# ltiao/bore

Measured on AMD Instinct MI355X. Metric: BO-iterations/sec (fit+argmax), 16-16-1 MLP, higher is better.
Workload: dtype f32; 1 GPU; BASELINE config 4 (= config 1 x independent loops): Branin-2D, 16-16-1 MLP, q=0.25, 200 epochs, batch 64, 3 L-BFGS-B restarts from 1024 samples; loops_per_gpu=512, total_loops=512, schedule=async, N_start=15, N_end=217, parallelism=replica-shard x1

## Files before the change

### bore_amd/csrc/bore_engine.hip

```cpp
#include <hip/hip_runtime.h>

#include <chrono>
#include <cmath>
#include <cstdint>
#include <cstdlib>
#include <cstring>
#include <atomic>
#include <initializer_list>
#include <mutex>
#include <new>
#include <thread>
#include <vector>

#include <sched.h>

#include "../../include/bore_hip.h"
#include "host_common.h"

namespace {

struct Mt19937 {
  uint32_t key[624];
  int pos;
  uint32_t next32() {
    if (pos >= 624) {
      int i;
      for (i = 0; i < 624 - 397; ++i) {
        const uint32_t y = (key[i] & 0x80000000u) | (key[i + 1] & 0x7fffffffu);
        key[i] = key[i + 397] ^ (y >> 1) ^ (-(int32_t)(y & 1) & 0x9908b0dfu);
      }
      for (; i < 623; ++i) {
        const uint32_t y = (key[i] & 0x80000000u) | (key[i + 1] & 0x7fffffffu);
        key[i] = key[i + (397 - 624)] ^ (y >> 1) ^ (-(int32_t)(y & 1) & 0x9908b0dfu);
      }
      const uint32_t y = (key[623] & 0x80000000u) | (key[0] & 0x7fffffffu);
      key[623] = key[396] ^ (y >> 1) ^ (-(int32_t)(y & 1) & 0x9908b0dfu);
      pos = 0;
    }
    uint32_t y = key[pos++];
    y ^= (y >> 11);
    y ^= (y << 7) & 0x9d2c5680u;
    y ^= (y << 15) & 0xefc60000u;
    y ^= (y >> 18);
    return y;
  }
  double next_double() {
    const uint32_t a = next32() >> 5, b = next32() >> 6;
    return (a * 67108864.0 + b) / 9007199254740992.0;
  }
};

struct Group {
  int a = 0, b = 0;
  hipStream_t stream = nullptr;
  hipEvent_t done = nullptr, ev[4] = {nullptr, nullptr, nullptr, nullptr};
  int64_t n = 0, cap = 0;
  int64_t epochs_seen = 0, draws = 0, steps = 0;
  bool inflight = false, has_new = false;
  double *X_seen = nullptr, *y_seen = nullptr, *y_dense = nullptr;
  float *X32 = nullptr, *z = nullptr;
  double *new_x = nullptr, *new_y = nullptr;
  double *x0 = nullptr, *x = nullptr, *jac = nullptr, *fun = nullptr, *x_best = nullptr;
  int32_t *idx = nullptr, *info = nullptr, *best = nullptr;
  double *new_x_pin = nullptr, *new_y_pin = nullptr, *x_best_pin = nullptr;
  int32_t *best_pin = nullptr, *info_pin = nullptr;
};

struct Async {
  int64_t cap = 0;
  IterEngine eng = {};
  double *result = nullptr;
  int32_t *flag = nullptr;
  int64_t *stamps = nullptr;
  double ns_per_tick = 10.0;
  std::vector<int32_t> it, target, state;
  std::vector<double> x_new, y_new, ready_since;
  std::vector<double> seen_at;
  double *ynew = nullptr;
  int32_t *yseq = nullptr, *parked = nullptr;
  int32_t *abort_flag = nullptr;
  int64_t wait_ticks = 0;
  std::vector<uint8_t> via_launch;
  std::vector<Worker> workers;
  std::vector<int> scratch_ids, done_ids;
  std::vector<double> cb_x, cb_y;
  bool fused = false;
  bool queue = false;
  QueueEntry *q_ring = nullptr;
  unsigned long long *q_head = nullptr, q_tail = 0;
  unsigned long long *q_tail_host = nullptr;
  int q_mask = 0, q_wgs = 0;
  int per_cu = 0;
  int host_threads = 1;
  int32_t *d_ident = nullptr;
  std::vector<int> q_owner;
  long long n_resident = 0, n_parked = 0;
  int stream_concurrency = 0;
  std::vector<double> launched_at;
  std::vector<double> loop_acc;
  double sum_wait = 0, sum_flight = 0;
  long long n_wait = 0, n_batches = 0, n_slots = 0;
};

}

__global__ void bore_spin_kernel(long long ticks) {
  const long long t0 = wall_clock64();
  while (wall_clock64() - t0 < ticks) __builtin_amdgcn_s_sleep(8);
}

extern "C" int bore_objective_branin01(const double *x, int64_t n, int32_t D, double *y, void *) {
  if (D != 2 || !x || !y) return 1;
  const double pi = 3.141592653589793;
  const double a = 5.1 / (4 * (pi * pi)), b = 5 / pi, c = 10 * (1 - 1 / (8 * pi));
  for (int64_t i = 0; i < n; ++i) {
    const double x1 = 15.0 * x[2 * i] - 5.0, x2 = 15.0 * x[2 * i + 1];
    const double t = x2 - a * (x1 * x1) + b * x1 - 6;
    y[i] = t * t + c * std::cos(x1) + 10;
  }
  return 0;
}

struct bore_engine {
  bore_mlp_desc desc;
  bore_engine_cfg cfg;
  int D = 0, P = 0;
  std::vector<double> low, high;
  bore_objective_fn objective = nullptr;
  void *user = nullptr;
  float *theta = nullptr, *adam_m = nullptr, *adam_v = nullptr;
  int64_t *adam_t = nullptr;
  std::vector<Mt19937> rs;
  std::vector<Group> groups;
  bore_engine_stats st;
  std::vector<double> y_tmp;
  Async *as = nullptr;
  bool poisoned = false;
};

namespace {

double now_s() {
  return std::chrono::duration<double>(std::chrono::steady_clock::now().time_since_epoch()).count();
}

template <typename T>
int dev_alloc(T **p, size_t count) {
  HIP_TRY(hipMalloc(reinterpret_cast<void **>(p), count * sizeof(T)));
  return 0;
}
template <typename T>
int pin_alloc(T **p, size_t count) {
  HIP_TRY(hipHostMalloc(reinterpret_cast<void **>(p), count * sizeof(T), hipHostMallocDefault));
  return 0;
// ... 218 lines not shown
  return 0;
}

int async_create(bore_engine *e, const double *X0, const double *y0) {
  const size_t L = e->cfg.n_loops, D = e->D, R = e->cfg.num_starts, n0 = e->cfg.n_init;
  if (R > 16) return fail(BORE_E_UNSUPPORTED, "engine_create: async_loops needs num_starts <= 16");
  e->as = new (std::nothrow) Async();
  if (!e->as) return fail(BORE_E_HIP, "engine_create: out of memory");
  Async &A = *e->as;
  int rc;
  if ((rc = async_alloc(e, n0 * 2 > 128 ? n0 * 2 : 128))) return rc;
  {
    const bore_engine_cfg &c = e->cfg;
    IterEngine &E = A.eng;
    E.desc = &e->desc; E.theta = e->theta; E.adam_m = e->adam_m; E.adam_v = e->adam_v; E.adam_t = e->adam_t;
    E.gamma = c.gamma; E.epochs = c.epochs; E.batch_size = c.batch_size; E.seed = c.seed; E.loop_id0 = c.loop_id0;
    E.adam = &c.adam; E.num_samples = c.num_samples; E.low = e->low.data(); E.high = e->high.data();
    E.num_starts = c.num_starts; E.transform = c.transform; E.opts = &c.lbfgsb; E.n_loops = c.n_loops;
  }
  std::vector<float> x32(L * n0 * D);
  for (size_t i = 0; i < x32.size(); ++i) x32[i] = (float)X0[i];
  HIP_TRY(hipMemcpy2D(A.eng.X_seen, A.cap * D * 8, X0, n0 * D * 8, n0 * D * 8, L, hipMemcpyHostToDevice));
  HIP_TRY(hipMemcpy2D(A.eng.y_seen, A.cap * 8, y0, n0 * 8, n0 * 8, L, hipMemcpyHostToDevice));
  HIP_TRY(hipMemcpy2D(A.eng.X32, A.cap * D * 4, x32.data(), n0 * D * 4, n0 * D * 4, L, hipMemcpyHostToDevice));
  if ((rc = pin_alloc(&A.result, L * (D + 8))) || (rc = pin_alloc(&A.flag, L)) ||
      (rc = dev_alloc(&A.stamps, L * 4)))
    return rc;
  std::memset(A.flag, 0, L * 4);
  HIP_TRY(hipMemset(A.stamps, 0, L * 4 * 8));
  {
    int dev = 0, khz = 0;
    HIP_TRY(hipGetDevice(&dev));
    if (hipDeviceGetAttribute(&khz, hipDeviceAttributeWallClockRate, dev) == hipSuccess && khz > 0)
      A.ns_per_tick = 1e6 / khz;
  }
  A.seen_at.assign(L, 0.0);
  A.via_launch.assign(L, 1);
  {
    char *blk = nullptr;
    const size_t bytes = L * (D + 1) * 8 + (2 * L + 1) * 4;
    if ((rc = pin_alloc(&blk, bytes))) return rc;
    std::memset(blk, 0, bytes);
    A.ynew = reinterpret_cast<double *>(blk);
    A.yseq = reinterpret_cast<int32_t *>(blk + L * (D + 1) * 8);
    A.parked = A.yseq + L;
    A.abort_flag = A.parked + L;
    for (size_t l = 0; l < L; ++l) A.parked[l] = -1;
  }
  A.it.assign(L, 0); A.target.assign(L, 0); A.state.assign(L, 2);
  A.x_new.assign(L * D, 0.0); A.y_new.assign(L, 0.0); A.ready_since.assign(L, 0.0);
  A.scratch_ids.reserve(L); A.cb_x.resize(L * D); A.cb_y.resize(L);
  A.launched_at.assign(L, 0.0);
  A.done_ids.assign(L, 0);
  A.fused = iteration_shape(&e->desc) != 0;
  const double resident_us = e->cfg.resident_wait_us < 0 ? 2000.0 : (double)e->cfg.resident_wait_us;
  A.wait_ticks = A.fused && resident_us > 0 ? (int64_t)(resident_us * 1e3 / A.ns_per_tick) : 0;
  const int queues = getenv("GPU_MAX_HW_QUEUES") ? atoi(getenv("GPU_MAX_HW_QUEUES")) : 4;
  int n_workers = A.fused ? 12 : 4;
  if (A.fused && n_workers > queues - 2) n_workers = queues - 2 > 2 ? queues - 2 : 2;
  if (e->cfg.worker_streams > 0) n_workers = e->cfg.worker_streams;
  A.workers.resize(n_workers > 0 ? n_workers : 1);
  for (Worker &w : A.workers) {
    HIP_TRY(hipStreamCreateWithFlags(&w.stream, hipStreamNonBlocking));
    HIP_TRY(hipEventCreateWithFlags(&w.done, hipEventDisableTiming));
    for (hipEvent_t &ev : w.ev) HIP_TRY(hipEventCreate(&ev));
    w.stage_bytes = ((sizeof(IterArgs) + 15) & ~(size_t)15) + L * (D + 1) * 8 + 3 * L * 4;
    char *hb = nullptr, *db = nullptr;
    if ((rc = pin_alloc(&hb, w.stage_bytes)) || (rc = dev_alloc(&db, w.stage_bytes))) return rc;
    const size_t o_dbl = (sizeof(IterArgs) + 15) & ~(size_t)15, o_int = o_dbl + L * (D + 1) * 8;
    w.h_args = reinterpret_cast<IterArgs *>(hb); w.d_args = reinterpret_cast<IterArgs *>(db);
    w.h_dbl = reinterpret_cast<double *>(hb + o_dbl); w.d_dbl = reinterpret_cast<double *>(db + o_dbl);
    w.h_int = reinterpret_cast<int32_t *>(hb + o_int); w.d_int = reinterpret_cast<int32_t *>(db + o_int);
    if ((rc = dev_alloc(&w.x0, L * R * D)) || (rc = dev_alloc(&w.x, L * R * D)) ||
        (rc = dev_alloc(&w.jac, L * R * D)) || (rc = dev_alloc(&w.fun, L * R)) ||
        (rc = dev_alloc(&w.idx, L * R)) || (rc = dev_alloc(&w.info, L * R * 5)))
      return rc;
  }
  if (A.workers.size() > 1) {
    const long long ticks = (long long)(2e6 / A.ns_per_tick);
    hipLaunchKernelGGL(bore_spin_kernel, dim3(1), dim3(64), 0, A.workers[0].stream, 1000LL);
    HIP_TRY(hipStreamSynchronize(A.workers[0].stream));
    double t0 = now_s();
    hipLaunchKernelGGL(bore_spin_kernel, dim3(1), dim3(64), 0, A.workers[0].stream, ticks);
    HIP_TRY(hipStreamSynchronize(A.workers[0].stream));
    const double one = now_s() - t0;
    t0 = now_s();
    for (Worker &w : A.workers) hipLaunchKernelGGL(bore_spin_kernel, dim3(1), dim3(64), 0, w.stream, ticks);
    for (Worker &w : A.workers) HIP_TRY(hipStreamSynchronize(w.stream));
    const double dt = now_s() - t0;
    int conc = (int)A.workers.size();
    if (dt > 1.5 * one) conc = (int)(A.workers.size() * one / dt + 0.5);
    conc = conc < 1 ? 1 : (conc > (int)A.workers.size() ? (int)A.workers.size() : conc);
    A.stream_concurrency = conc;
    if (conc < (int)A.workers.size()) {
      if (queues < (int)A.workers.size() + 2)
        fprintf(stderr,
                "bore_engine: %zu worker streams, but the device ran only about %d of them at once (one 2-ms probe "
                "alone %.2f ms, %zu at once %.2f ms): streams share hardware queues.  Set GPU_MAX_HW_QUEUES >= %zu in "
                "the environment BEFORE the first GPU call of the process (it is %d now).\n",
                A.workers.size(), conc, 1e3 * one, A.workers.size(), 1e3 * dt, A.workers.size() + 2, queues);
      else if (getenv("BORE_ASYNC_DEBUG"))
        fprintf(stderr,
                "bore_engine: stream probe: one 2-ms probe alone %.2f ms, %zu at once %.2f ms -> about %d run side by "
                "side (GPU_MAX_HW_QUEUES = %d already covers the %zu streams: not a queue shortage)\n",
                1e3 * one, A.workers.size(), 1e3 * dt, conc, queues, A.workers.size());
    }
  }
  return async_decide_schedule(e);
}

void async_destroy(bore_engine *e) {
  if (!e->as) return;
  Async &A = *e->as;
  for (Worker &w : A.workers) {
    free_all({w.d_args, w.x0, w.x, w.jac, w.fun, w.idx, w.info}, {w.h_args});
    free_stream(w.stream, w.done, w.ev);
  }
  free_all({A.eng.X_seen, A.eng.y_seen, A.eng.X32, A.eng.z, A.stamps, A.q_head, A.d_ident},
           {A.result, A.flag, A.ynew, A.q_ring, A.q_tail_host});
  delete e->as;
  e->as = nullptr;
}

int async_enqueue(bore_engine *e, Worker &w, int B, int64_t N_max) {
  const IterEngine &E = e->as->eng;
  void *sp = w.stream;
  int rc;
  if (e->as->fused) {
    if ((rc = record_event(w.ev[2], w.stream)) || (rc = iteration_launch(E, w, B)) || (rc = record_event(w.ev[3], w.stream)))
      return rc;
    return record_event(w.done, w.stream);
  }
  if ((rc = bore_append_observations(B, e->D, E.X_seen, E.y_seen, 0, e->as->cap, w.d_dbl,
                                     w.d_dbl + (size_t)E.n_loops * e->D, E.X32, nullptr, sp)) ||
      (rc = bore_labels(B, E.y_seen, N_max, E.gamma, E.z, nullptr, sp)) || (rc = record_event(w.ev[0], w.stream)) ||
      (rc = bore_mlp_fit(E.desc, B, E.theta, E.adam_m, E.adam_v, E.adam_t, E.X32, E.z, N_max, E.epochs, E.batch_size,
                         nullptr, E.seed, E.loop_id0, 0, E.adam, nullptr, sp)) ||
      (rc = record_event(w.ev[1], w.stream)) ||
      (rc = bore_sample_screen_topk(E.desc, B, E.theta, E.seed, E.loop_id0, 0, E.num_samples, E.low, E.high,
                                    E.num_starts, w.x0, w.idx, nullptr, sp)) ||
      (rc = record_event(w.ev[2], w.stream)) ||
      (rc = bore_lbfgsb_minimize(E.desc, B, E.theta, E.transform, 1, w.x0, E.num_starts, E.low, E.high, E.opts, w.x,
                                 w.fun, w.jac, w.info, sp)) ||
      (rc = record_event(w.ev[3], w.stream)))
    return rc;
  return record_event(w.done, w.stream);
}

int async_launch(bore_engine *e, Worker &w) {
  const double t0 = now_s();
  Async &A = *e->as;
  const bore_engine_cfg &c = e->cfg;
  const int L = c.n_loops, D = e->D, B = (int)A.scratch_ids.size();
  int max_it = 0;
  double *hx = w.h_dbl, *hy = w.h_dbl + (size_t)L * D;
  for (int b = 0; b < B; ++b) {
    const int l = A.scratch_ids[b], it = A.it[l];
    w.h_int[b] = l;
    w.h_int[L + b] = it;
    w.h_int[2 * L + b] = A.target[l];
    std::memcpy(hx + (size_t)b * D, &A.x_new[(size_t)l * D], (size_t)D * 8);
    hy[b] = A.y_new[l];
    max_it = it > max_it ? it : max_it;
    A.state[l] = 1;
    A.via_launch[l] = 1;
    A.launched_at[l] = t0;
    A.sum_wait += t0 - A.ready_since[l];
    e->st.ready_to_launch_s += t0 - A.ready_since[l];
    ++A.n_wait;
    __atomic_store_n(&A.parked[l], -1, __ATOMIC_RELAXED);
    __atomic_store_n(&A.yseq[l], it, __ATOMIC_RELEASE);
  }
  if (!A.fused)
    HIP_TRY(hipMemcpyAsync(w.d_dbl, w.h_dbl, w.stage_bytes - ((sizeof(IterArgs) + 15) & ~(size_t)15),
                           hipMemcpyHostToDevice, w.stream));
  const bore_batch bt = async_batch(e, w.d_int, w.d_int + L, w.d_int + 2 * L, A.fused);
  bore_set_batch(&bt);
  const int rc = async_enqueue(e, w, B, c.n_init + max_it);
  bore_set_batch(nullptr);
  if (rc) return rc;
  w.busy = true;
  ++A.n_batches;
  ++e->st.batches;
  A.n_slots += B;
  e->st.host_enqueue_s += now_s() - t0;
  return 0;
}

int retire_worker(bore_engine *e, Worker &w) {
  float ms = 0.f;
  if (!e->as->fused) {
    HIP_TRY(hipEventElapsedTime(&ms, w.ev[0], w.ev[1]));
    e->st.fit_ms += ms;
  }
  e->st.fit_launches += 1;
  HIP_TRY(hipEventElapsedTime(&ms, w.ev[2], w.ev[3]));
  e->st.argmax_ms += ms;
  e->st.argmax_launches += 1;
  w.busy = false;
  return 0;
}

int async_drain(bore_engine *e) {
  __atomic_store_n(e->as->abort_flag, 1, __ATOMIC_RELEASE);
  for (Worker &w : e->as->workers) {
    (void)hipStreamSynchronize(w.stream);
    w.busy = false;
  }
  __atomic_store_n(e->as->abort_flag, 0, __ATOMIC_RELEASE);
  e->poisoned = true;
  return 0;
}

static int take_async_result(bore_engine *e, int l, double t0, int n_done, bore_engine_stats &st, double &sum_flight,
                             double *xbuf, int *ids) {
  Async &A = *e->as;
  const bore_engine_cfg &c = e->cfg;
  const int L = c.n_loops, D = e->D;
  A.state[l] = 3;
  const double *r = A.result + (size_t)l * (D + 8);
  double *xn = xbuf + (size_t)n_done * D;
  sum_flight += t0 - A.launched_at[l];
  A.seen_at[l] = t0;
  st.launch_to_result_s += t0 - A.launched_at[l];
  st.phase_ns_labels += r[D + 3] * A.ns_per_tick;
  st.phase_ns_fit += r[D + 4] * A.ns_per_tick;
  st.phase_ns_screen += r[D + 5] * A.ns_per_tick;
  st.phase_ns_lbfgsb += r[D + 6] * A.ns_per_tick;
  ++st.phase_iterations;
  if (A.loop_acc.size() == (size_t)L * 6) {
    double *la = &A.loop_acc[(size_t)l * 6];
    la[0] += r[D + 4] * A.ns_per_tick; la[1] += r[D + 6] * A.ns_per_tick;
    la[2] += r[D + 1]; la[3] += r[D + 2]; la[4] += t0 - A.launched_at[l]; la[5] += 1.0;
  }
  if (r[D] < 0.0) {
    ++st.none_results;
    Mt19937 &rs = e->rs[l];
    for (int d = 0; d < D; ++d) xn[d] = e->low[d] + (e->high[d] - e->low[d]) * rs.next_double();
  } else {
    std::memcpy(xn, r, (size_t)D * 8);
  }
  st.n_fg_rows += (int64_t)r[D + 7];
  st.n_fg_requests += (int64_t)r[D + 1];
  st.n_rounds += (int64_t)r[D + 2];
  st.argmax_bytes += r[D + 7] * 4.0 * (2 * D + 1) + r[D + 2] * 4.0 * e->P;
  const double N = c.n_init + A.it[l], steps = std::ceil(N / c.batch_size);
  st.fit_bytes += c.epochs * (4.0 * N * (D + 1) + steps * 24.0 * e->P);
  ids[n_done++] = l;
  return n_done;
}

static int async_host_threads(const bore_engine *e, int L) {
  int cores = (int)std::thread::hardware_concurrency();
  cpu_set_t set;
  if (sched_getaffinity(0, sizeof(set), &set) == 0) cores = CPU_COUNT(&set);
  int t = L / 8192 + 1;
  if (t > 4) t = 4;
  if (t > cores - 1) t = cores - 1;
  (void)e;
  return t < 1 ? 1 : t;
}

static int async_run_queue(bore_engine *e, int n_steps) {
  Async &A = *e->as;
  const bore_engine_cfg &c = e->cfg;
  const int L = c.n_loops, D = e->D;
  Worker &w = A.workers[0];
  const size_t ring_n = (size_t)A.q_mask + 1;
  std::memset(A.q_ring, 0, ring_n * sizeof(QueueEntry));
  A.q_tail = 0;
  A.q_owner.assign(ring_n * 2, -1);
  HIP_TRY(hipMemsetAsync(A.q_head, 0, 2 * sizeof(unsigned long long), w.stream));
  __atomic_store_n(A.q_tail_host, 0ull, __ATOMIC_RELEASE);
  std::atomic<int> stop{0};
  auto push = [&](int lid, int it) {
    const unsigned long long t = __atomic_fetch_add(&A.q_tail, 1ull, __ATOMIC_RELAXED);
    const size_t slot = (size_t)(t & (unsigned long long)A.q_mask);
    int *own = &A.q_owner[slot * 2];
    const int old_lid = __atomic_load_n(&own[0], __ATOMIC_ACQUIRE), old_it = own[1];
    if (old_lid >= 0) {
      const double t0 = now_s();
      while (__atomic_load_n(&A.flag[old_lid], __ATOMIC_ACQUIRE) < old_it + 1 && !stop.load(std::memory_order_relaxed))
// ... 96 lines not shown
      } else if (t0 - last_progress > 30.0) {
        stop.store(2);
      }
    }
  };
  {
    std::vector<std::thread> helpers;
    for (int ti = 1; ti < T; ++ti) helpers.emplace_back(serve, ti);
    serve(0);
    for (std::thread &th : helpers) th.join();
  }
  for (const Share &sh : shares) {
    const bore_engine_stats &p = sh.st;
    bore_engine_stats &q = e->st;
    q.launch_to_result_s += p.launch_to_result_s; q.result_to_ready_s += p.result_to_ready_s;
    q.phase_ns_labels += p.phase_ns_labels; q.phase_ns_fit += p.phase_ns_fit; q.phase_ns_screen += p.phase_ns_screen;
    q.phase_ns_lbfgsb += p.phase_ns_lbfgsb; q.phase_iterations += p.phase_iterations; q.none_results += p.none_results;
    q.n_fg_rows += p.n_fg_rows; q.n_fg_requests += p.n_fg_requests; q.n_rounds += p.n_rounds;
    q.argmax_bytes += p.argmax_bytes; q.fit_bytes += p.fit_bytes;
    A.sum_flight += sh.sum_flight;
    A.n_resident += sh.n_resident;
  }
  {
    double busiest = 0;
    for (const Share &sh : shares) busiest = sh.st.host_finalize_s > busiest ? sh.st.host_finalize_s : busiest;
    e->st.host_finalize_s += busiest;
  }
  if (stop.load()) {
    const int why = stop.load();
    __atomic_store_n(A.q_tail_host, ~0ull, __ATOMIC_RELEASE);
    async_drain(e);
    for (int l = 0; l < L; ++l) A.state[l] = 2;
    return why == 1 ? fail(BORE_E_CALLBACK, "engine_run: the objective callback failed")
                    : fail(BORE_E_HIP, "engine_run: no loop finished for 30 s");
  }
  __atomic_store_n(A.q_tail_host, ~0ull, __ATOMIC_RELEASE);
  HIP_TRY(hipStreamSynchronize(w.stream));
  return retire_worker(e, w);
}

int async_run(bore_engine *e, int n_steps) {
  Async &A = *e->as;
  const bore_engine_cfg &c = e->cfg;
  const int L = c.n_loops, D = e->D;
  int max_it = 0;
  for (int l = 0; l < L; ++l) max_it = A.it[l] > max_it ? A.it[l] : max_it;
  int rc;
  if (c.n_init + max_it + n_steps > A.cap) {
    int64_t cap = A.cap;
    while (cap < c.n_init + max_it + n_steps) cap *= 2;
    if ((rc = async_alloc(e, cap)) || (rc = async_decide_schedule(e))) return rc;
  }
  if (A.queue) return async_run_queue(e, n_steps);
  const double start = now_s();
  int remaining = L;
  for (int l = 0; l < L; ++l) {
    A.target[l] = A.it[l] + n_steps;
    A.state[l] = 0;
    A.ready_since[l] = start;
  }
  const bool resident = A.fused && A.wait_ticks > 0;
  const int min_batch = resident ? 1 : (L >= 16 ? L / 8 : 1);
  const double max_wait = resident ? 0.0 : 150e-6;
  double last_progress = start, first_done = start;
  int n_done = 0;
  const int cb_min = resident ? 1 : (L >= 64 ? L / 16 : 1);
  const double cb_wait = resident ? 0.0 : 40e-6;
  while (remaining) {
    const double t0 = now_s();
    for (int l = 0; l < L; ++l) {
      if (A.state[l] != 1) continue;
      if (__atomic_load_n(&A.flag[l], __ATOMIC_ACQUIRE) != A.it[l] + 1) {
        if (A.fused && !A.via_launch[l] && __atomic_load_n(&A.parked[l], __ATOMIC_ACQUIRE) == A.it[l]) {
          A.state[l] = 0;
          A.ready_since[l] = t0;
          ++A.n_parked;
        }
        continue;
      }
      if (n_done == 0) first_done = t0;
      n_done = take_async_result(e, l, t0, n_done, e->st, A.sum_flight, A.cb_x.data(), A.done_ids.data());
    }
    if (n_done && (n_done >= cb_min || t0 - first_done >= cb_wait)) {
      if (e->objective(A.cb_x.data(), n_done, D, A.cb_y.data(), e->user)) {
        async_drain(e);
        for (int l = 0; l < L; ++l) A.state[l] = 2;
        return fail(BORE_E_CALLBACK, "engine_run: the objective callback failed");
      }
      const double now = now_s();
      for (int k = 0; k < n_done; ++k) {
        const int l = A.done_ids[k];
        std::memcpy(&A.x_new[(size_t)l * D], &A.cb_x[(size_t)k * D], (size_t)D * 8);
        A.y_new[l] = A.cb_y[k];
        e->st.result_to_ready_s += now - A.seen_at[l];
        ++A.it[l];
        if (A.it[l] >= A.target[l]) {
          A.state[l] = 2;
          --remaining;
        } else if (A.fused) {
          double *yn = A.ynew + (size_t)l * (D + 1);
          std::memcpy(yn, &A.cb_x[(size_t)k * D], (size_t)D * 8);
          yn[D] = A.cb_y[k];
          __atomic_store_n(&A.yseq[l], A.it[l], __ATOMIC_RELEASE);
          A.state[l] = 1;
          A.via_launch[l] = 0;
          A.launched_at[l] = now;
// ... 234 lines not shown
  if (e->as) {
    Async &A = *e->as;
    const size_t L = e->cfg.n_loops;
    HIP_TRY(hipDeviceSynchronize());
    const int64_t nd = A.it[0] > 0 ? N - 1 : N;
    HIP_TRY(hipMemcpy2D(X, (size_t)N * D * 8, A.eng.X_seen, A.cap * D * 8, (size_t)nd * D * 8, L,
                        hipMemcpyDeviceToHost));
    HIP_TRY(hipMemcpy2D(y, (size_t)N * 8, A.eng.y_seen, A.cap * 8, (size_t)nd * 8, L, hipMemcpyDeviceToHost));
    if (A.it[0] > 0)
      for (size_t l = 0; l < L; ++l) {
        std::memcpy(X + (l * N + nd) * D, &A.x_new[l * D], (size_t)D * 8);
        y[l * N + nd] = A.y_new[l];
      }
    return 0;
  }
  for (Group &g : e->groups) {
    const size_t Lg = g.b - g.a;
    HIP_TRY(hipStreamSynchronize(g.stream));
    HIP_TRY(hipMemcpy2D(X + (size_t)g.a * N * D, (size_t)N * D * 8, g.X_seen, g.cap * D * 8,
                        (size_t)g.n * D * 8, Lg, hipMemcpyDeviceToHost));
    HIP_TRY(hipMemcpy2D(y + (size_t)g.a * N, (size_t)N * 8, g.y_seen, g.cap * 8, (size_t)g.n * 8, Lg,
                        hipMemcpyDeviceToHost));
    if (g.has_new)
      for (size_t l = 0; l < Lg; ++l) {
        std::memcpy(X + ((size_t)(g.a + l) * N + g.n) * D, g.new_x_pin + l * D, (size_t)D * 8);
        y[(size_t)(g.a + l) * N + g.n] = g.new_y_pin[l];
      }
  }
  return 0;
}

extern "C" int bore_engine_state(bore_engine *e, float *theta, float *adam_m, float *adam_v,
                                 int64_t *adam_t) {
  if (!e) return fail(BORE_E_INVALID, "engine_state: NULL engine");
  if (e->poisoned) return fail(BORE_E_INVALID, kPoisoned);
  HIP_TRY(hipDeviceSynchronize());
  const size_t n = (size_t)e->cfg.n_loops * e->P;
  if (theta) HIP_TRY(hipMemcpy(theta, e->theta, n * 4, hipMemcpyDeviceToHost));
  if (adam_m) HIP_TRY(hipMemcpy(adam_m, e->adam_m, n * 4, hipMemcpyDeviceToHost));
  if (adam_v) HIP_TRY(hipMemcpy(adam_v, e->adam_v, n * 4, hipMemcpyDeviceToHost));
  if (adam_t) HIP_TRY(hipMemcpy(adam_t, e->adam_t, (size_t)e->cfg.n_loops * 8, hipMemcpyDeviceToHost));
  return 0;
}

extern "C" int bore_debug_engine_loop_stats(bore_engine *e, double *out, int reset) {
  if (!e || !e->as) return fail(BORE_E_INVALID, "loop_stats: an asynchronous engine is needed");
  Async &A = *e->as;
  const size_t n = (size_t)e->cfg.n_loops * 6;
  if (out && A.loop_acc.size() == n) std::memcpy(out, A.loop_acc.data(), n * 8);
  if (reset) A.loop_acc.assign(n, 0.0);
  return 0;
}

extern "C" int bore_engine_get_stats(bore_engine *e, bore_engine_stats *out, int reset) {
  if (!e || !out) return fail(BORE_E_INVALID, "engine_get_stats: NULL argument");
  *out = e->st;
  out->worker_streams = e->as ? (int64_t)e->as->workers.size() : (int64_t)e->groups.size();
  out->stream_concurrency = e->as ? e->as->stream_concurrency : 0;
  out->loops_per_cu = e->as ? e->as->per_cu : 0;
  out->side_by_side_workgroups = e->as && e->as->fused ? (e->as->queue ? e->as->q_wgs : e->cfg.n_loops) : 0;
  out->host_threads = e->as ? e->as->host_threads : 1;
  if (reset) std::memset(&e->st, 0, sizeof(e->st));
  return 0;
}
```

### bore_amd/csrc/bore_iter.hip

```cpp

struct QueueEntry {
  int lid, it;
};

struct IterArgs {
  FitArgs f;
  ScreenArgs s;
  LbfgsbArgs b;
  double *X_seen, *y_seen;
  float *X32, *z;
  const double *x_new, *y_new;
  long long *stamps;
  double gamma;
  int D;
  const int *targets;
  const double *ynew;
  const int *yseq;
  int *parked;
  const int *abort_flag;
  long long wait_ticks;
  const QueueEntry *q_ring;
  unsigned long long *q_head;
  int q_mask;
  const unsigned long long *q_tail_host;
  int progress;
};

__device__ __forceinline__ double load_host_f64(const double *p) {
  const long long v = __hip_atomic_load(reinterpret_cast<const long long *>(p), __ATOMIC_RELAXED,
                                        __HIP_MEMORY_SCOPE_SYSTEM);
  return __longlong_as_double(v);
}

#define BORE_LAG_YIELD_Q 3
__device__ __forceinline__ void phase_handoff() {
  __builtin_amdgcn_fence(__ATOMIC_RELEASE, "workgroup");
  asm volatile("s_waitcnt vmcnt(0) lgkmcnt(0)" ::: "memory");
  __syncthreads();
  __builtin_amdgcn_fence(__ATOMIC_ACQUIRE, "workgroup");
  asm volatile("buffer_inv sc0\n\ts_waitcnt vmcnt(0)" ::: "memory");
}

template <int SHAPE, bool LOCAL = false>
__device__ __forceinline__ void iteration_once(const IterArgs *__restrict__ pa,
                                                         const long long slot, const int it,
                                                         const bool staged, const long long t_begin = 0) {
  const IterArgs &a = *pa;
  const long long lid = uniform_i64(a.f.ids[slot]), cap = a.f.cap;
  long long *stp = a.stamps ? a.stamps + lid * 4 : nullptr;
  if (stp && threadIdx.x == 0) stp[0] = t_begin ? t_begin : wall_clock64();
  if (it > 0) {
    const long long row = a.f.n_init + it - 1;
    for (int d = threadIdx.x; d < a.D; d += blockDim.x) {
      const double v = staged ? a.x_new[slot * a.D + d] : load_host_f64(a.ynew + lid * (a.D + 1) + d);
      a.X_seen[(lid * cap + row) * a.D + d] = v;
      a.X32[(lid * cap + row) * a.D + d] = (float)v;
    }
    if (threadIdx.x == 0)
      a.y_seen[lid * cap + row] = staged ? a.y_new[slot] : load_host_f64(a.ynew + lid * (a.D + 1) + a.D);
  }
  if constexpr (LOCAL) phase_handoff();
  else {
    __threadfence();
    __syncthreads();
  }
  labels_body(a.y_seen, 0, 0.0, a.z, nullptr, a.f.ids, a.f.its, a.f.n_init, cap, a.gamma, slot, it);
  if (stp && threadIdx.x == 0) stp[1] = wall_clock64();
  if constexpr (LOCAL) phase_handoff();
  else {
    __threadfence();
    __syncthreads();
  }
  fit_body<SHAPE>(a.f, slot, it);
  if (stp && threadIdx.x == 0) stp[2] = wall_clock64();
  if constexpr (LOCAL) phase_handoff();
  else {
    __threadfence();
    __syncthreads();
  }
  screen_body<SHAPE, false>(a.s, slot, it);
  if (stp && threadIdx.x == 0) stp[3] = wall_clock64();
  if constexpr (LOCAL) phase_handoff();
  else {
    __threadfence();
    __syncthreads();
  }
  lbfgsb_body<SHAPE, false, true, true, false, LOCAL ? 1 : 0>(a.b, slot, 0, it);
}

template <int SHAPE, bool RESIDENT, int OCC = 2>
__global__ __launch_bounds__(BORE_THREADS, OCC) void iteration_kernel(const IterArgs *__restrict__ pa) {
  const long long slot = blockIdx.x;
  const int it_first = uniform_i32(pa->f.its[slot]);
  if constexpr (!RESIDENT) {
    typedef const __attribute__((address_space(4))) IterArgs *IterArgsConst1;
    const IterArgs &a = *(const IterArgs *)(IterArgsConst1) reinterpret_cast<unsigned long long>(pa);
    const long long lid = uniform_i64(a.f.ids[slot]), cap = a.f.cap;
    const int it = it_first;
    long long *stp = a.stamps ? a.stamps + lid * 4 : nullptr;
    if (stp && threadIdx.x == 0) stp[0] = wall_clock64();
    if (it > 0) {
      const long long row = a.f.n_init + it - 1;
      for (int d = threadIdx.x; d < a.D; d += blockDim.x) {
        const double v = a.x_new[slot * a.D + d];
        a.X_seen[(lid * cap + row) * a.D + d] = v;
        a.X32[(lid * cap + row) * a.D + d] = (float)v;
      }
      if (threadIdx.x == 0) a.y_seen[lid * cap + row] = a.y_new[slot];
    }
    __threadfence();
    __syncthreads();
    labels_body(a.y_seen, 0, 0.0, a.z, nullptr, a.f.ids, a.f.its, a.f.n_init, cap, a.gamma, slot);
    if (stp && threadIdx.x == 0) stp[1] = wall_clock64();
    __threadfence();
    __syncthreads();
    fit_body<SHAPE>(a.f, slot);
    if (stp && threadIdx.x == 0) stp[2] = wall_clock64();
    __threadfence();
    __syncthreads();
    screen_body<SHAPE, false>(a.s, slot);
    if (stp && threadIdx.x == 0) stp[3] = wall_clock64();
    __threadfence();
    __syncthreads();
    lbfgsb_body<SHAPE, false, true, true, false>(a.b, slot, 0);
    if (a.targets && threadIdx.x == 0 && it + 1 < a.targets[slot])
      __hip_atomic_store(a.parked + lid, it + 1, __ATOMIC_RELEASE, __HIP_MEMORY_SCOPE_SYSTEM);
    return;
  }
  __shared__ __attribute__((aligned(16))) int s_go4[4];
  const int target = pa->targets ? uniform_i32(pa->targets[slot]) : it_first + 1;
  int *prog;
  {
    unsigned long long pb = reinterpret_cast<unsigned long long>(pa) + offsetof(IterArgs, progress);
    asm volatile("" : "+s"(pb));
    prog = reinterpret_cast<int *>(pb);
  }
  for (int it = it_first;;) {
    {
      const int total = __hip_atomic_load(prog, __ATOMIC_RELAXED, __HIP_MEMORY_SCOPE_AGENT);
      const int n_wg = (int)gridDim.x;
      const int lead = uniform_i32((it - it_first) * n_wg - total);
      if (lead < -(n_wg >> 1)) __builtin_amdgcn_s_setprio(3);
      else if (lead > (n_wg >> 1)) __builtin_amdgcn_s_setprio(0);
      else __builtin_amdgcn_s_setprio(1);
    }
    unsigned long long pa_bits = reinterpret_cast<unsigned long long>(pa);
    asm volatile("" : "+s"(pa_bits));
    typedef const __attribute__((address_space(4))) IterArgs *IterArgsConst;
    iteration_once<SHAPE, true>((const IterArgs *)(IterArgsConst)pa_bits, slot, it, it == it_first);
    __syncthreads();
    ++it;
    if (threadIdx.x == 0) __hip_atomic_fetch_add(prog, 1, __ATOMIC_RELAXED, __HIP_MEMORY_SCOPE_AGENT);
    if (it >= target) break;
    if (threadIdx.x == 0) {
      const long long lid = pa->f.ids[slot], wait_ticks = pa->wait_ticks;
      const int *yseq = pa->yseq + lid, *abort_flag = pa->abort_flag;
      int go = 0;
      const long long t0 = wall_clock64();
      for (;;) {
        if (__hip_atomic_load(yseq, __ATOMIC_RELAXED, __HIP_MEMORY_SCOPE_SYSTEM) >= it) {
          asm volatile("" ::: "memory");
          go = 1;
          break;
        }
        if (wait_ticks <= 0 || wall_clock64() - t0 > wait_ticks) break;
        if (__hip_atomic_load(abort_flag, __ATOMIC_RELAXED, __HIP_MEMORY_SCOPE_SYSTEM)) break;
        __builtin_amdgcn_s_sleep(16);
      }
      if (go) {
        const long long t1 = wall_clock64();
        const int n_wg = (int)gridDim.x;
        for (;;) {
          const int total = __hip_atomic_load(prog, __ATOMIC_RELAXED, __HIP_MEMORY_SCOPE_AGENT);
          if (4 * ((it - it_first) * n_wg - total) <= BORE_LAG_YIELD_Q * n_wg || wall_clock64() - t1 > 50000) break;
          __builtin_amdgcn_s_sleep(64);
        }
      }
      if (!go) __hip_atomic_store(pa->parked + lid, it, __ATOMIC_RELEASE, __HIP_MEMORY_SCOPE_SYSTEM);
      s_go4[0] = go;
    }
    __syncthreads();
    const int go = uniform_i32(s_go4[0]);
// ... 81 lines not shown
  if (desc->compute != BORE_COMPUTE_F32) return 0;
  const int f = bore_kernel_flavour(desc, true);
  if (f == 1) return 1;
  if (f == 5 && desc->input_dim == 16 && bore_flavour_on(5)) return 5;
  return 0;
}

static constexpr bool fused_flavour_on(int shape) { return shape == 1 || bore_flavour_on(shape); }
static constexpr int fused_most_per_cu(int shape) { return shape == 5 ? 2 : 3; }

static int iteration_loops_per_cu(int shape, size_t lds_bytes, int *per_cu_out) {
  static thread_local size_t seen_bytes = ~(size_t)0;
  static thread_local int seen_per_cu = 0, seen_dev = -1, seen_shape = 0;
  int dev = 0;
  HIP_TRY(hipGetDevice(&dev));
  if (seen_bytes != lds_bytes || seen_dev != dev || seen_shape != shape) {
    int per_cu = 0, q_per_cu = 0;
    const int most = fused_most_per_cu(shape);
    const int rc = bore_with_flavour<fused_flavour_on>(FlavourList<5, 1>{}, shape, [&](auto S) {
      constexpr int OCC = fused_most_per_cu(S());
      HIP_TRY(hipOccupancyMaxActiveBlocksPerMultiprocessor(&per_cu, iteration_kernel<S(), true, OCC>, BORE_THREADS, lds_bytes));
      HIP_TRY(hipOccupancyMaxActiveBlocksPerMultiprocessor(&q_per_cu, queue_kernel<S(), OCC>, BORE_THREADS, lds_bytes));
      return 0;
    });
    if (rc) return rc;
    if (q_per_cu < per_cu) per_cu = q_per_cu;
    const size_t granule = 1280, static_bytes = 16;
    const size_t each = (lds_bytes + static_bytes + granule - 1) / granule * granule;
    const int by_lds = (int)(BORE_LDS_BYTES / each);
    if (by_lds < per_cu) per_cu = by_lds;
    if (per_cu > most) per_cu = most;
    seen_bytes = lds_bytes; seen_dev = dev; seen_per_cu = per_cu; seen_shape = shape;
  }
  *per_cu_out = seen_per_cu;
  return 0;
}

struct IterEngine {
  const bore_mlp_desc *desc;
  float *theta, *adam_m, *adam_v;
  int64_t *adam_t;
  double *X_seen, *y_seen;
  float *X32, *z;
  double gamma;
  int epochs, batch_size;
  uint64_t seed;
  int64_t loop_id0;
  const bore_adam_cfg *adam;
  int64_t num_samples;
  const double *low, *high;
  int num_starts, transform;
  const bore_lbfgsb_opts *opts;
  int n_loops;
};

struct Worker {
  hipStream_t stream = nullptr;
  hipEvent_t done = nullptr, ev[4] = {nullptr, nullptr, nullptr, nullptr};
  bool busy = false;
  int32_t *h_int = nullptr, *d_int = nullptr;
  double *h_dbl = nullptr, *d_dbl = nullptr;
  double *x0 = nullptr, *x = nullptr, *jac = nullptr, *fun = nullptr;
  int32_t *idx = nullptr, *info = nullptr;
  IterArgs *h_args = nullptr, *d_args = nullptr;
  size_t stage_bytes = 0;
};

struct IterQueue {
  const QueueEntry *ring;
  unsigned long long *head;
  int mask;
  const unsigned long long *tail_host;
  int wgs;
};

struct IterPlan {
  int shape;
  size_t lds_bytes;
  size_t part_bytes[4];
};

static int iteration_plan(const IterEngine &E, const Worker &w, int n_slots, IterArgs *h, IterPlan *plan) {
  if (!g_batch) return fail(BORE_E_INVALID, "iteration_launch: no batch set");
  const int64_t cap = g_batch->cap;
  size_t lf = 0, ls = 0, lb = 0;
  int sf = 0, ss = 0, sb = 0, blocks = 0;
  int rc = fit_build(E.desc, n_slots, E.theta, E.adam_m, E.adam_v, E.adam_t, E.X32, E.z, cap, E.epochs, E.batch_size,
                     nullptr, E.seed, E.loop_id0, 0, E.adam, nullptr, h->f, lf, sf);
  if (rc) return rc < 0 ? rc : fail(BORE_E_INVALID, "iteration_launch: epochs must be positive");
  const SampleSpec spec{E.seed, E.loop_id0, 0, E.low, E.high};
  if ((rc = screen_build(E.desc, n_slots, E.theta, nullptr, &spec, E.num_samples, 0, E.num_starts, w.x0, w.idx,
                         nullptr, h->s, ls, ss)))
    return rc;
  if ((rc = lbfgsb_build(E.desc, n_slots, E.theta, E.transform, 1, w.x0, E.num_starts, E.low, E.high, E.opts, w.x,
                         w.fun, w.jac, w.info, h->b, lb, sb, blocks)))
    return rc;
  const int shape = iteration_shape(E.desc);
  if (!shape || sf != shape || ss != shape || sb != shape || blocks != 1)
    return fail(BORE_E_UNSUPPORTED, "iteration_launch: static shape 1, or 5 at 16 inputs, one workgroup per loop");
  h->X_seen = E.X_seen; h->y_seen = E.y_seen; h->X32 = E.X32; h->z = E.z;
  h->x_new = w.d_dbl; h->y_new = w.d_dbl + (size_t)E.n_loops * E.desc->input_dim;
  h->stamps = reinterpret_cast<long long *>(g_batch->stamps);
  h->b.stamps = h->stamps;
  h->targets = g_batch->targets;
  h->ynew = g_batch->ynew; h->yseq = g_batch->yseq; h->parked = g_batch->parked;
  h->abort_flag = g_batch->abort_flag;
  const bool resident = g_batch->targets && g_batch->ynew && g_batch->yseq && g_batch->parked &&
                        g_batch->abort_flag;
  if (!resident) h->targets = nullptr;
  h->wait_ticks = resident ? g_batch->wait_ticks : 0;
  h->gamma = E.gamma;
  h->D = E.desc->input_dim;
  h->progress = 0;
  h->q_ring = nullptr; h->q_head = nullptr; h->q_mask = 0; h->q_tail_host = nullptr;
  size_t floats = lf > ls ? lf : ls;
  floats = floats > lb ? floats : lb;
  const size_t labels_floats = 2 * ((size_t)cap + 2);
  floats = floats > labels_floats ? floats : labels_floats;
  *plan = IterPlan{shape, floats * 4, {lf * 4, ls * 4, lb * 4, labels_floats * 4}};
  return bore_with_flavour<fused_flavour_on>(FusedFlavours{}, shape, [&](auto S) {
    int rc = 0;
    if ((rc = allow_lds(iteration_kernel<S(), true, 2>, floats * 4)) || (rc = allow_lds(iteration_kernel<S(), false, 2>, floats * 4)) ||
        (rc = allow_lds(queue_kernel<S(), 2>, floats * 4)))
      return rc;
    if constexpr (fused_most_per_cu(S()) == 3)
      if ((rc = allow_lds(iteration_kernel<S(), true, 3>, floats * 4)) || (rc = allow_lds(queue_kernel<S(), 3>, floats * 4))) return rc;
    return 0;
  });
}

template <typename K>
static int fused_launch(K kernel, int workgroups, const IterPlan &p, const Worker &w) {
  hipLaunchKernelGGL(kernel, dim3(workgroups), dim3(BORE_THREADS), p.lds_bytes, w.stream, (const IterArgs *)w.d_args);
  HIP_TRY(hipGetLastError());
  return 0;
}

static int iteration_launch_queue(const IterEngine &E, Worker &w, int n_slots, const IterQueue &q) {
  IterArgs *h = w.h_args;
  IterPlan p;
  if (const int rc = iteration_plan(E, w, n_slots, h, &p)) return rc;
  if (q.wgs < 1 || !q.ring || !q.head || !q.tail_host || !g_batch->ynew || !g_batch->abort_flag)
    return fail(BORE_E_INVALID, "iteration_launch: incomplete work queue");
  h->q_ring = q.ring; h->q_head = q.head; h->q_mask = q.mask; h->q_tail_host = q.tail_host;
  h->targets = nullptr;
  h->wait_ticks = 0;
  HIP_TRY(hipMemcpyAsync(w.d_args, h, sizeof(IterArgs), hipMemcpyHostToDevice, w.stream));
  return bore_with_flavour<fused_flavour_on>(FusedFlavours{}, p.shape, [&](auto S) {
    if constexpr (fused_most_per_cu(S()) == 3)
      if (q.wgs > 2 * device_cus()) return fused_launch(queue_kernel<S(), 3>, q.wgs, p, w);
    return fused_launch(queue_kernel<S(), 2>, q.wgs, p, w);
  });
}

static int iteration_launch(const IterEngine &E, Worker &w, int n_slots) {
  IterArgs *h = w.h_args;
  IterPlan p;
  int rc;
  if ((rc = iteration_plan(E, w, n_slots, h, &p))) return rc;
  if (h->wait_ticks > 0) {
    int per_cu = 0;
    if ((rc = iteration_loops_per_cu(p.shape, p.lds_bytes, &per_cu))) return rc;
    if (getenv("BORE_ASYNC_DEBUG"))
      fprintf(stderr, "[bore] fused kernel: %zu B of LDS per loop (fit %zu, screen %zu, restarts %zu, labels %zu), %d loops per CU\n",
              p.lds_bytes, p.part_bytes[0], p.part_bytes[1], p.part_bytes[2], p.part_bytes[3], per_cu);
    if (g_batch->resident_loops > per_cu * device_cus()) h->wait_ticks = 0;
  }
  HIP_TRY(hipMemcpyAsync(w.d_args, h, w.stage_bytes, hipMemcpyHostToDevice, w.stream));
  return bore_with_flavour<fused_flavour_on>(FusedFlavours{}, p.shape, [&](auto S) {
    if constexpr (fused_most_per_cu(S()) == 3)
      if (h->wait_ticks > 0 && g_batch->resident_loops > 2 * device_cus()) return fused_launch(iteration_kernel<S(), true, 3>, n_slots, p, w);
    if (h->wait_ticks > 0) return fused_launch(iteration_kernel<S(), true, 2>, n_slots, p, w);
    return fused_launch(iteration_kernel<S(), false, 2>, n_slots, p, w);
  });
}
```

### bore_amd/engine.py

```python
from __future__ import annotations

import time

import ctypes as _lib_ctypes

import numpy as np
import torch

from . import _lib, ops
from .optimizers import lockstep
from .transforms import resolve


def branin01(X):
    x1, x2 = 15.0 * X[..., 0] - 5.0, 15.0 * X[..., 1]
    return ((x2 - 5.1 / (4 * np.pi ** 2) * x1 ** 2 + 5 / np.pi * x1 - 6) ** 2
            + 10 * (1 - 1 / (8 * np.pi)) * np.cos(x1) + 10)


def initial_state(loop_ids, D, units, P, n_init, objective, low, high):
    rss = [np.random.RandomState(int(s)) for s in loop_ids]
    th = np.empty((len(rss), P), dtype=np.float32)
    for i, rs in enumerate(rss):
        off, fan_in = 0, D
# ... 107 lines not shown
                _lib.lib().bore_engine_destroy(h)

    def __del__(self):
        try:
            self.close()
        except Exception:
            pass

    def run(self, n_steps):
        with _RUN_LOCK:
            _RUN_DEPTH[0] += 1
        try:
            rc = _lib.lib().bore_engine_run(self._h, int(n_steps))
        finally:
            with _RUN_LOCK:
                _RUN_DEPTH[0] -= 1
                late = [_DEFERRED.pop() for _ in range(len(_DEFERRED))] if _RUN_DEPTH[0] == 0 else []
            for h in late:
                _lib.lib().bore_engine_destroy(h)
        if self._error is not None:
            e, self._error = self._error, None
            raise e
        _lib.check(rc)

    @property
    def N(self):
        return int(_lib.lib().bore_engine_size(self._h))

    def observations(self):
        N = self.N
        X, y = np.empty((self.L, N, self.D)), np.empty((self.L, N))
        vp = lambda a: a.ctypes.data_as(_lib_ctypes.c_void_p)
        _lib.check(_lib.lib().bore_engine_observations(self._h, vp(X), vp(y)))
        return X, y

    @property
    def X(self):
        return self.observations()[0]

    @property
    def y(self):
        return self.observations()[1]

    def state(self):
        th, m, v = (np.empty((self.L, self.P), dtype=np.float32) for _ in range(3))
        t = np.empty(self.L, dtype=np.int64)
        vp = lambda a: a.ctypes.data_as(_lib_ctypes.c_void_p)
        _lib.check(_lib.lib().bore_engine_state(self._h, vp(th), vp(m), vp(v), vp(t)))
        return th, m, v, t

    def take_stats(self, reset=True):
        st = _lib.EngineStats()
        _lib.check(_lib.lib().bore_engine_get_stats(self._h, _lib_ctypes.byref(st), int(reset)))
        return {k: getattr(st, k) for k, _ in st._fields_}

    def best(self):
        X, y = self.observations()
        i = np.argmin(y, axis=1)
        return X[np.arange(self.L), i], y[np.arange(self.L), i]




class ShardedEngine:

    def __init__(self, loop_ids, shards=2, **kw):
        ids = np.asarray(loop_ids, dtype=np.int64)
        shards = int(max(1, min(shards, len(ids))))
        if shards > 1:
            kw = dict(kw, resident_wait_us=0, worker_streams=max(2, 12 // shards), work_queue=False)
        self.engines = [NativeEngine(part, **kw) for part in np.array_split(ids, shards)]
        e0 = self.engines[0]
        self.loop_ids, self.L, self.D, self.P = ids, len(ids), e0.D, e0.P
        self.n_groups = e0.n_groups
        self.device = e0.device

    def run(self, n_steps):
        import threading
        errors = []

        def work(eng):
            try:
                torch.cuda.set_device(eng.device)
                eng.run(n_steps)
            except BaseException as err:
                errors.append(err)

        threads = [threading.Thread(target=work, args=(e,)) for e in self.engines[1:]]
        for t in threads:
            t.start()
        work(self.engines[0])
        for t in threads:
            t.join()
        if errors:
            raise errors[0]

    def close(self):
        for e in self.engines:
            e.close()

    @property
    def N(self):
        return self.engines[0].N

    def observations(self):
        parts = [e.observations() for e in self.engines]
        return np.concatenate([p[0] for p in parts]), np.concatenate([p[1] for p in parts])

    @property
    def X(self):
        return self.observations()[0]

    @property
    def y(self):
        return self.observations()[1]

    def state(self):
        parts = [e.state() for e in self.engines]
        return tuple(np.concatenate([p[i] for p in parts]) for i in range(4))

    def take_stats(self, reset=True):
        stats = [e.take_stats(reset) for e in self.engines]
        out = {k: sum(s[k] for s in stats) for k in stats[0]}
        out["stream_concurrency"] = min(s["stream_concurrency"] for s in stats)
        out["loops_per_cu"] = min(s["loops_per_cu"] for s in stats)
        return out

    def best(self):
        X, y = self.observations()
        i = np.argmin(y, axis=1)
        return X[np.arange(self.L), i], y[np.arange(self.L), i]


class ReplicaEngine:

    def __init__(self, loop_ids, input_dim=2, units=(16, 16, 1), acts=("relu", "relu", "sigmoid"),
                 transform="identity", gamma=0.25, epochs=200, batch_size=64, num_starts=3,
                 num_samples=1024, n_init=10, objective=branin01, max_points=None,
                 options=None, device=None, mode="device", seed=0, groups=1, select="device",
                 deduplicate=False):
        assert mode in ("device", "lockstep")
        assert select in ("device", "host")
        self.select, self.deduplicate = select, bool(deduplicate)
        self.mode, self.seed = mode, int(seed)
        self.device = device or _lib.require_gpu()
        self.loop_ids = np.asarray(loop_ids, dtype=np.int64)
        self.L = L = len(self.loop_ids)
        assert L >= 1 and np.array_equal(self.loop_ids, self.loop_ids[0] + np.arange(L)), \
            "loop ids must be consecutive (the device streams are keyed by first id + offset)"
        self.D = D = int(input_dim)
        self.units, self.acts = list(units), list(acts)
        self.desc = _lib.make_desc(D, self.units, self.acts)
        self.P = ops.param_count(self.desc)
        self.transform = resolve(transform)
        assert self.transform.name is not None, "the replica engine runs on the device only: a named transform"
        self.gamma, self.epochs, self.batch_size = gamma, int(epochs), int(batch_size)
        self.num_starts, self.num_samples = int(num_starts), int(num_samples)
        self.objective = objective
        self.options = dict(options or dict(maxiter=1000, ftol=1e-9))
        self.low, self.high = np.zeros(D), np.ones(D)
        self.rs, th, X0, y0 = initial_state(self.loop_ids, D, self.units, self.P, n_init,
                                            self.objective, self.low, self.high)
        self.theta = torch.from_numpy(th).to(self.device)
        self.adam_m = torch.zeros_like(self.theta)
        self.adam_v = torch.zeros_like(self.theta)
        self.adam_t = torch.zeros(L, dtype=torch.int64, device=self.device)
        self._lo, self._lo_p = ops._host_f64(self.low, D, "low")
        self._hi, self._hi_p = ops._host_f64(self.high, D, "high")
        self._adam = _lib.AdamCfg(1e-3, 0.9, 0.999, 1e-7)
        self._lopts = lbfgsb_opts(self.options)
        G = max(1, min(int(groups), L)) if mode == "device" else 1
        bounds = np.linspace(0, L, G + 1).astype(int)
        self.groups = [_Group(int(a), int(b), X0[a:b], y0[a:b], self)
                       for a, b in zip(bounds[:-1], bounds[1:])]
        self.stats = dict(fit_ms=[], fit_bytes=[], argmax_ms=[], argmax_bytes=[], n_fg_rows=0,
                          n_rounds=0, none_results=0)
        self._ev, self._ev2 = [], []

# ... 323 lines not shown
```

Measured before the change: 292,800 BO-iterations/s.

## Pair heavy and light loops on each CU using cost-sorted slot placement

The host keeps a running average of per-loop iteration cost in ticks and sorts each batch's loops from heaviest to lightest. In the resident fused kernel, each workgroup reads its hardware CU and XCC id and takes a slot through atomic counters keyed by CU. The first tenant on a CU takes the next heavy slot from the front, and later tenants take light slots from the back. The aim is to even out per-CU work so the slowest CU finishes sooner, at the cost of extra atomics, a slightly larger staging copy, and debug statistics in take_stats.

```diff
diff --git a/bore_amd/csrc/bore_engine.hip b/bore_amd/csrc/bore_engine.hip
--- a/bore_amd/csrc/bore_engine.hip
+++ b/bore_amd/csrc/bore_engine.hip
@@ -5,11 +5,13 @@
 #include <cstdint>
 #include <cstdlib>
 #include <cstring>
+#include <algorithm>
 #include <atomic>
 #include <initializer_list>
 #include <mutex>
 #include <new>
 #include <thread>
+#include <utility>
 #include <vector>
 
 #include <sched.h>
@@ -100,6 +102,10 @@
   std::vector<double> loop_acc;
   double sum_wait = 0, sum_flight = 0;
   long long n_wait = 0, n_batches = 0, n_slots = 0;
+  std::vector<double> cost;
+  std::vector<double> placed_cost;
+  std::vector<std::pair<double, int>> order;
+  int placed_worker = -1, placed_slots = 0;
 };
 
 }
@@ -424,6 +430,14 @@
   A.scratch_ids.reserve(L); A.cb_x.resize(L * D); A.cb_y.resize(L);
   A.launched_at.assign(L, 0.0);
   A.done_ids.assign(L, 0);
+  A.cost.assign(L, 0.0);
+  A.placed_cost.assign(L, 0.0);
+  A.order.reserve(L);
+  A.eng.place_fold = getenv("BORE_PLACEMENT") && !atoi(getenv("BORE_PLACEMENT")) ? -1 : 0;
+  if (A.eng.place_fold == 0 && getenv("BORE_PLACEMENT_FOLD")) {
+    const int fold = atoi(getenv("BORE_PLACEMENT_FOLD"));
+    A.eng.place_fold = fold < 0 ? 0 : (fold > BORE_PLACE_KEYS ? BORE_PLACE_KEYS : fold);
+  }
   A.fused = iteration_shape(&e->desc) != 0;
   const double resident_us = e->cfg.resident_wait_us < 0 ? 2000.0 : (double)e->cfg.resident_wait_us;
   A.wait_ticks = A.fused && resident_us > 0 ? (int64_t)(resident_us * 1e3 / A.ns_per_tick) : 0;
@@ -436,10 +450,13 @@
     HIP_TRY(hipStreamCreateWithFlags(&w.stream, hipStreamNonBlocking));
     HIP_TRY(hipEventCreateWithFlags(&w.done, hipEventDisableTiming));
     for (hipEvent_t &ev : w.ev) HIP_TRY(hipEventCreate(&ev));
-    w.stage_bytes = ((sizeof(IterArgs) + 15) & ~(size_t)15) + L * (D + 1) * 8 + 3 * L * 4;
+    const size_t o_dbl = (sizeof(IterArgs) + 15) & ~(size_t)15, o_int = o_dbl + L * (D + 1) * 8, o_place = o_int + 3 * L * 4;
+    w.stage_bytes = o_place + (2 + BORE_PLACE_KEYS) * 4;
     char *hb = nullptr, *db = nullptr;
     if ((rc = pin_alloc(&hb, w.stage_bytes)) || (rc = dev_alloc(&db, w.stage_bytes))) return rc;
-    const size_t o_dbl = (sizeof(IterArgs) + 15) & ~(size_t)15, o_int = o_dbl + L * (D + 1) * 8;
+    std::memset(hb, 0, w.stage_bytes);
+    w.d_place = reinterpret_cast<int32_t *>(db + o_place);
+    if ((rc = dev_alloc(&w.d_place_slots, (size_t)BORE_PLACE_KEYS * BORE_PLACE_RANKS))) return rc;
     w.h_args = reinterpret_cast<IterArgs *>(hb); w.d_args = reinterpret_cast<IterArgs *>(db);
     w.h_dbl = reinterpret_cast<double *>(hb + o_dbl); w.d_dbl = reinterpret_cast<double *>(db + o_dbl);
     w.h_int = reinterpret_cast<int32_t *>(hb + o_int); w.d_int = reinterpret_cast<int32_t *>(db + o_int);
@@ -485,7 +502,7 @@
   if (!e->as) return;
   Async &A = *e->as;
   for (Worker &w : A.workers) {
-    free_all({w.d_args, w.x0, w.x, w.jac, w.fun, w.idx, w.info}, {w.h_args});
+    free_all({w.d_args, w.x0, w.x, w.jac, w.fun, w.idx, w.info, w.d_place_slots}, {w.h_args});
     free_stream(w.stream, w.done, w.ev);
   }
   free_all({A.eng.X_seen, A.eng.y_seen, A.eng.X32, A.eng.z, A.stamps, A.q_head, A.d_ident},
@@ -526,6 +543,22 @@
   const int L = c.n_loops, D = e->D, B = (int)A.scratch_ids.size();
   int max_it = 0;
   double *hx = w.h_dbl, *hy = w.h_dbl + (size_t)L * D;
+  if (A.fused && A.wait_ticks > 0 && A.eng.place_fold >= 0) {
+    double sum = 0.0;
+    int known = 0;
+    for (const int l : A.scratch_ids)
+      if (A.cost[l] > 0.0) {
+        sum += A.cost[l];
+        ++known;
+      }
+    const double mean = known ? sum / known : 0.0;
+    A.order.clear();
+    for (const int l : A.scratch_ids) A.order.emplace_back(A.cost[l] > 0.0 ? A.cost[l] : mean, l);
+    if (known)
+      std::stable_sort(A.order.begin(), A.order.end(),
+                       [](const std::pair<double, int> &p, const std::pair<double, int> &q) { return p.first > q.first; });
+    for (int b = 0; b < B; ++b) A.scratch_ids[b] = A.order[b].second;
+  }
   for (int b = 0; b < B; ++b) {
     const int l = A.scratch_ids[b], it = A.it[l];
     w.h_int[b] = l;
@@ -551,6 +584,15 @@
   const int rc = async_enqueue(e, w, B, c.n_init + max_it);
   bore_set_batch(nullptr);
   if (rc) return rc;
+  const int wi = (int)(&w - A.workers.data());
+  if (w.placed && B >= A.placed_slots) {
+    A.placed_worker = wi;
+    A.placed_slots = B;
+    for (int b = 0; b < B; ++b) A.placed_cost[(size_t)b] = A.order[(size_t)b].first;
+  } else if (wi == A.placed_worker) {
+    A.placed_worker = -1;
+    A.placed_slots = 0;
+  }
   w.busy = true;
   ++A.n_batches;
   ++e->st.batches;
@@ -600,6 +642,10 @@
   st.phase_ns_screen += r[D + 5] * A.ns_per_tick;
   st.phase_ns_lbfgsb += r[D + 6] * A.ns_per_tick;
   ++st.phase_iterations;
+  {
+    const double ticks = r[D + 3] + r[D + 4] + r[D + 5] + r[D + 6];
+    A.cost[l] = A.cost[l] > 0.0 ? A.cost[l] + 0.25 * (ticks - A.cost[l]) : ticks;
+  }
   if (A.loop_acc.size() == (size_t)L * 6) {
     double *la = &A.loop_acc[(size_t)l * 6];
     la[0] += r[D + 4] * A.ns_per_tick; la[1] += r[D + 6] * A.ns_per_tick;
@@ -802,6 +848,8 @@
     if ((rc = async_alloc(e, cap)) || (rc = async_decide_schedule(e))) return rc;
   }
   if (A.queue) return async_run_queue(e, n_steps);
+  A.placed_worker = -1;
+  A.placed_slots = 0;
   const double start = now_s();
   int remaining = L;
   for (int l = 0; l < L; ++l) {
@@ -1142,6 +1190,38 @@
   return 0;
 }
 
+extern "C" int bore_debug_engine_placement(bore_engine *e, double *out) {
+  if (!e || !out) return fail(BORE_E_INVALID, "engine_placement: NULL argument");
+  for (int k = 0; k < 8; ++k) out[k] = 0.0;
+  if (!e->as || e->as->placed_worker < 0) return 0;
+  Async &A = *e->as;
+  const Worker &w = A.workers[(size_t)A.placed_worker];
+  std::vector<int32_t> tab(2 + BORE_PLACE_KEYS), slots((size_t)BORE_PLACE_KEYS * BORE_PLACE_RANKS);
+  HIP_TRY(hipStreamSynchronize(w.stream));
+  HIP_TRY(hipMemcpy(tab.data(), w.d_place, tab.size() * 4, hipMemcpyDeviceToHost));
+  HIP_TRY(hipMemcpy(slots.data(), w.d_place_slots, slots.size() * 4, hipMemcpyDeviceToHost));
+  for (int key = 0; key < BORE_PLACE_KEYS; ++key) {
+    const int n = tab[(size_t)2 + key];
+    if (n < 1) continue;
+    out[n >= 3 ? 2 : n - 1] += 1.0;
+    double sum = 0.0;
+    for (int r = 0; r < n && r < BORE_PLACE_RANKS; ++r) {
+      const int s = slots[(size_t)key * BORE_PLACE_RANKS + r];
+      if (s >= 0 && s < A.placed_slots) sum += A.placed_cost[(size_t)s];
+    }
+    out[3] = sum * A.ns_per_tick > out[3] ? sum * A.ns_per_tick : out[3];
+    if (n == 2) {
+      const int off = slots[(size_t)key * BORE_PLACE_RANKS] + slots[(size_t)key * BORE_PLACE_RANKS + 1] - (A.placed_slots - 1);
+      out[6] += off == 0 ? 1.0 : 0.0;
+      out[7] += off < 0 ? -off : off;
+    }
+  }
+  if (out[1] > 0.0) out[7] /= out[1];
+  out[4] = A.placed_slots;
+  out[5] = tab[0];
+  return 0;
+}
+
 extern "C" int bore_engine_get_stats(bore_engine *e, bore_engine_stats *out, int reset) {
   if (!e || !out) return fail(BORE_E_INVALID, "engine_get_stats: NULL argument");
   *out = e->st;
diff --git a/bore_amd/csrc/bore_iter.hip b/bore_amd/csrc/bore_iter.hip
--- a/bore_amd/csrc/bore_iter.hip
+++ b/bore_amd/csrc/bore_iter.hip
@@ -24,7 +24,12 @@
   int q_mask;
   const unsigned long long *q_tail_host;
   int progress;
-};
+  int *place, *place_slots;
+  int place_fold;
+};
+
+#define BORE_PLACE_KEYS 2048
+#define BORE_PLACE_RANKS 4
 
 __device__ __forceinline__ double load_host_f64(const double *p) {
   const long long v = __hip_atomic_load(reinterpret_cast<const long long *>(p), __ATOMIC_RELAXED,
@@ -90,7 +95,31 @@
 
 template <int SHAPE, bool RESIDENT, int OCC = 2>
 __global__ __launch_bounds__(BORE_THREADS, OCC) void iteration_kernel(const IterArgs *__restrict__ pa) {
-  const long long slot = blockIdx.x;
+  __shared__ __attribute__((aligned(16))) int s_go4[4];
+  unsigned slot32 = blockIdx.x;
+  if constexpr (RESIDENT) {
+    int *place = pa->place;
+    if (place) {
+      if (threadIdx.x == 0) {
+        const unsigned hw = __builtin_amdgcn_s_getreg((4) | (0 << 6) | (31 << 11));
+        const unsigned xcc = __builtin_amdgcn_s_getreg((20) | (0 << 6) | (31 << 11));
+        unsigned key = ((xcc & 7u) << 8) | ((hw >> 8) & 0xffu);
+        const int fold = pa->place_fold;
+        if (fold > 0) key %= (unsigned)fold;
+        const int n = (int)gridDim.x;
+        const int rank = __hip_atomic_fetch_add(place + 2 + key, 1, __ATOMIC_RELAXED, __HIP_MEMORY_SCOPE_AGENT);
+        int s = rank == 0 ? __hip_atomic_fetch_add(place, 1, __ATOMIC_RELAXED, __HIP_MEMORY_SCOPE_AGENT)
+                          : n - 1 - __hip_atomic_fetch_add(place + 1, 1, __ATOMIC_RELAXED, __HIP_MEMORY_SCOPE_AGENT);
+        if ((unsigned)s >= (unsigned)n) s = (int)blockIdx.x;
+        if (rank < BORE_PLACE_RANKS) pa->place_slots[key * BORE_PLACE_RANKS + rank] = s;
+        s_go4[1] = s;
+      }
+      __syncthreads();
+      slot32 = (unsigned)uniform_i32(s_go4[1]);
+    }
+    asm volatile("" : "+s"(slot32));
+  }
+  const long long slot = slot32;
   const int it_first = uniform_i32(pa->f.its[slot]);
   if constexpr (!RESIDENT) {
     typedef const __attribute__((address_space(4))) IterArgs *IterArgsConst1;
@@ -127,7 +156,6 @@
       __hip_atomic_store(a.parked + lid, it + 1, __ATOMIC_RELEASE, __HIP_MEMORY_SCOPE_SYSTEM);
     return;
   }
-  __shared__ __attribute__((aligned(16))) int s_go4[4];
   const int target = pa->targets ? uniform_i32(pa->targets[slot]) : it_first + 1;
   int *prog;
   {
@@ -315,6 +343,7 @@
   int num_starts, transform;
   const bore_lbfgsb_opts *opts;
   int n_loops;
+  int place_fold;
 };
 
 struct Worker {
@@ -327,6 +356,8 @@
   int32_t *idx = nullptr, *info = nullptr;
   IterArgs *h_args = nullptr, *d_args = nullptr;
   size_t stage_bytes = 0;
+  int32_t *d_place = nullptr, *d_place_slots = nullptr;
+  bool placed = false;
 };
 
 struct IterQueue {
@@ -376,6 +407,7 @@
   h->D = E.desc->input_dim;
   h->progress = 0;
   h->q_ring = nullptr; h->q_head = nullptr; h->q_mask = 0; h->q_tail_host = nullptr;
+  h->place = nullptr; h->place_slots = nullptr; h->place_fold = 0;
   size_t floats = lf > ls ? lf : ls;
   floats = floats > lb ? floats : lb;
   const size_t labels_floats = 2 * ((size_t)cap + 2);
@@ -429,6 +461,10 @@
               p.lds_bytes, p.part_bytes[0], p.part_bytes[1], p.part_bytes[2], p.part_bytes[3], per_cu);
     if (g_batch->resident_loops > per_cu * device_cus()) h->wait_ticks = 0;
   }
+  w.placed = h->wait_ticks > 0 && E.place_fold >= 0 && w.d_place && w.d_place_slots;
+  if (w.placed) {
+    h->place = w.d_place; h->place_slots = w.d_place_slots; h->place_fold = E.place_fold;
+  }
   HIP_TRY(hipMemcpyAsync(w.d_args, h, w.stage_bytes, hipMemcpyHostToDevice, w.stream));
   return bore_with_flavour<fused_flavour_on>(FusedFlavours{}, p.shape, [&](auto S) {
     if constexpr (fused_most_per_cu(S()) == 3)
diff --git a/bore_amd/engine.py b/bore_amd/engine.py
--- a/bore_amd/engine.py
+++ b/bore_amd/engine.py
@@ -183,7 +183,17 @@
     def take_stats(self, reset=True):
         st = _lib.EngineStats()
         _lib.check(_lib.lib().bore_engine_get_stats(self._h, _lib_ctypes.byref(st), int(reset)))
-        return {k: getattr(st, k) for k, _ in st._fields_}
+        out = {k: getattr(st, k) for k, _ in st._fields_}
+        pl = (_lib_ctypes.c_double * 8)()
+        fn = getattr(_lib.lib(), "bore_debug_engine_placement", None)
+        if fn is not None:
+            fn.argtypes = [_lib_ctypes.c_void_p, _lib_ctypes.c_void_p]
+            _lib.check(fn(self._h, pl))
+        out.update(placement_cus_1=int(pl[0]), placement_cus_2=int(pl[1]), placement_cus_3=int(pl[2]),
+                   placement_max_cu_cost_us=1e-3 * pl[3], placement_workgroups=int(pl[4]),
+                   placement_first_tenants=int(pl[5]), placement_mirror_pairs=int(pl[6]),
+                   placement_mirror_offset=float(pl[7]))
+        return out
 
     def best(self):
         X, y = self.observations()
@@ -255,6 +265,7 @@
         out = {k: sum(s[k] for s in stats) for k in stats[0]}
         out["stream_concurrency"] = min(s["stream_concurrency"] for s in stats)
         out["loops_per_cu"] = min(s["loops_per_cu"] for s in stats)
+        out["placement_max_cu_cost_us"] = max(s["placement_max_cu_cost_us"] for s in stats)
         return out
 
     def best(self):
```

New measurement: 289,900 BO-iterations/s. -1.0%, worse.
